# maksimt/rri_nmf

Measured on AMD Instinct MI355X. Metric: RRI sweeps/sec and achieved HBM GB/s on dense X (n x d, rank k), higher is better.
Workload: dtype f64

## Files before the change

### include/rri_hip.h

```cpp
#ifndef RRI_HIP_H
#define RRI_HIP_H

#include <stdint.h>
#include <stddef.h>

#ifdef __cplusplus
extern "C" {
#endif

#define RRI_ABI_VERSION 1
#define RRI_GRAM_SLICES 8
#define RRI_MAX_K 1024

typedef struct rri_ctx rri_ctx;
typedef struct rri_comm rri_comm;
#define RRI_COMM_ID_BYTES 128

typedef int32_t rri_status;
enum {
    RRI_OK = 0,
    RRI_PAUSED = 1,
    RRI_ERR_INVALID = -1,
    RRI_ERR_HIP = -2,
    RRI_ERR_UNSUPPORTED = -3,
// ... 92 lines not shown
rri_status rri_get_X_scales(rri_ctx* ctx, double* row_out, double* col_out);
rri_status rri_csr_column_positive_counts(rri_ctx* ctx, double* df_out);
rri_status rri_csr_scale_X(rri_ctx* ctx, const double* col_scale, int32_t normalize_rows, int64_t* zero_rows_out);

rri_status rri_comm_unique_id(uint8_t* id_out );
rri_status rri_comm_create(rri_comm** out, const uint8_t* id, int32_t rank, int32_t world, int32_t device);
typedef int32_t (*rri_allreduce_fn)(void* user, double* buf, int64_t count);
typedef int32_t (*rri_allgather_fn)(void* user, const double* send, int64_t count, double* recv);
typedef int32_t (*rri_broadcast_fn)(void* user, double* buf, int64_t count, int32_t root);
rri_status rri_comm_create_host(rri_comm** out, int32_t rank, int32_t world, rri_allreduce_fn allreduce,
                                rri_allgather_fn allgather, rri_broadcast_fn broadcast, void* user);
rri_status rri_comm_destroy(rri_comm* comm);
rri_status rri_attach_comm(rri_ctx* ctx, rri_comm* comm, int64_t row_offset, int64_t n_global);
rri_status rri_comm_broadcast(rri_ctx* ctx, double* host, int64_t count, int32_t root);
rri_status rri_comm_allreduce_sum(rri_ctx* ctx, double* host, int64_t count);
rri_status rri_comm_stats(rri_ctx* ctx, int32_t* rank, int32_t* world, int64_t* allreduce_calls);

rri_status rri_reduce_buffer(rri_ctx* ctx, void** dev_ptr, int64_t* n_elems);
rri_status rri_bind_reduce_buffer(rri_ctx* ctx, void* dev_ptr, int64_t n_elems);
rri_status rri_topic_reduce_local(rri_ctx* ctx, int32_t t);
rri_status rri_reduce_read(rri_ctx* ctx, double* out, int64_t count);
rri_status rri_reduce_write(rri_ctx* ctx, const double* in, int64_t count);
rri_status rri_topic_finish(rri_ctx* ctx, int32_t t);
rri_status rri_topic_finish_w(rri_ctx* ctx, int32_t t);
rri_status rri_resid_row_argmax(rri_ctx* ctx, double* value, int64_t* local_row);
rri_status rri_reset_row(rri_ctx* ctx, int64_t local_row, double* row_out_host);
rri_status rri_poll(rri_ctx* ctx);
rri_status rri_objective_parts(rri_ctx* ctx, double out[3]);

rri_status rri_timing_enable(rri_ctx* ctx, int32_t on);
rri_status rri_timing_read(rri_ctx* ctx, int32_t kernel_id, int64_t* launches, double* total_ms);
rri_status rri_synchronize(rri_ctx* ctx);
rri_status rri_onchip_info(rri_ctx* ctx, int32_t* eligible, int64_t* launches);
#define RRI_LAYOUT_FIELDS 23
rri_status rri_layout_info(rri_ctx* ctx, int64_t* out, int32_t n);
rri_status rri_onchip_fallbacks(rri_ctx* ctx, int64_t* fallbacks);
rri_status rri_device_memory(int64_t* buffers, int64_t* bytes);
rri_status rri_debug_xcc(rri_ctx* ctx, int32_t* out, int32_t count);
rri_status rri_sweep_until(rri_ctx* ctx, int32_t n_sweeps, double obj_prev, double stop_scale, double* obj_hist,
                           int32_t* sweeps_done);
rri_status rri_bench_rank1_update(rri_ctx* ctx, int32_t reps, double* avg_ms);
rri_status rri_bench_stream_copy(rri_ctx* ctx, int32_t reps, double* avg_ms);

#ifdef __cplusplus
}
#endif
#endif
```

### rri_nmf_amd/_capi.py

```python
import ctypes as C
import os

_PKG = os.path.dirname(os.path.abspath(__file__))
LIB_PATH = os.environ.get('RRI_HIP_LIB', os.path.join(_PKG, 'lib', 'librri_hip.so'))

RRI_GRAM_SLICES = 8
RRI_LAYOUT_FIELDS = 23
RRI_MAX_K = 1024
RRI_OK, RRI_PAUSED = 0, 1
RRI_ERR_INVALID, RRI_ERR_HIP, RRI_ERR_UNSUPPORTED = -1, -2, -3
RRI_ERR_UNBOUNDED, RRI_ERR_W_COL_ZERO, RRI_ERR_NOT_IMPLEMENTED, RRI_ERR_COMM = -4, -5, -6, -7
RRI_COMM_ID_BYTES = 128
RRI_F32, RRI_F64, RRI_F16 = 0, 1, 2
RRI_U8 = 4
RRI_UNWEIGHTED, RRI_WEIGHTED_DENSE, RRI_WEIGHTED_SPARSE, RRI_UNWEIGHTED_RESIDUAL, RRI_UNWEIGHTED_SPARSE = 0, 1, 2, 3, 4
RESET_NONE, RESET_MAX_RESID_DOCUMENT, RESET_RANDOM = 0, 1, 2
EVENT_NONE, EVENT_RESET_T, EVENT_RESET_W = 0, 1, 2
ABI_VERSION = 1


class Params(C.Structure):
    _fields_ = [('fix_W', C.c_int32), ('fix_T', C.c_int32), ('project_T_each_iter', C.c_int32),
                ('has_t_row_sum', C.c_int32), ('has_w_row_sum', C.c_int32), ('reset_method', C.c_int32),
                ('resets_left', C.c_int32), ('reserved0', C.c_int32),
                ('t_row_sum', C.c_double), ('w_row_sum', C.c_double),
                ('reg_w_l1', C.c_double), ('reg_w_l2', C.c_double), ('reg_t_l1', C.c_double),
                ('reg_t_l2', C.c_double), ('eps_div', C.c_double)]


class Event(C.Structure):
    _fields_ = [('kind', C.c_int32), ('topic', C.c_int32), ('sweep', C.c_int32), ('resume_topic', C.c_int32)]


_P = C.c_void_p
_I32, _I64, _D = C.c_int32, C.c_int64, C.c_double
ALLREDUCE_FN = C.CFUNCTYPE(C.c_int32, C.c_void_p, C.POINTER(C.c_double), C.c_int64)
ALLGATHER_FN = C.CFUNCTYPE(C.c_int32, C.c_void_p, C.POINTER(C.c_double), C.c_int64, C.POINTER(C.c_double))
BROADCAST_FN = C.CFUNCTYPE(C.c_int32, C.c_void_p, C.POINTER(C.c_double), C.c_int64, C.c_int32)
PROTOTYPES = {
    'rri_abi_version': (C.c_uint32, []),
# ... 137 lines not shown
```

### rri_nmf_amd/csrc/rri_hip.hip

```cpp
#include <hip/hip_runtime.h>
#include <dlfcn.h>
#include <rccl/rccl.h>

#include <algorithm>
#include <atomic>
#include <chrono>
#include <cstdarg>
#include <cstdio>
#include <mutex>
#include <cstdlib>
#include <cstring>
#include <string>
#include <utility>
#include <vector>

#include "rri_hip.h"
#include "rri_pick.hpp"
#include "rri_kernels.hpp"
#include "rri_wrri_kernels.hpp"
#include "rri_sparse_kernels.hpp"
#include "rri_onchip_kernels.hpp"

using namespace rri;

// ... 142 lines not shown
        unsigned short* idx = nullptr;
        void* val = nullptr;
        int* perm = nullptr;
        SpWork* work = nullptr;
    } sp[2];
    bool sparse_x = false;
    SpWork* spx_work = nullptr;
    double* rowhat = nullptr;
    double* Cpart = nullptr;
    double* N2part = nullptr;
    unsigned* Mcols = nullptr;
    bool nw_mask = false;
    bool mcols_tried = false;
    double mask_density = 1.0;
    int cpart_rows = 0;
    bool wcorr = false;
    int wcorr_topic = 0, wcorr_nrb = 0;
    bool resid_fresh = false;
    bool dt_pending = false;
    bool explicit_resid = false;
    bool dw_pending = false;
    int dw_topic = 0;
    double* told = nullptr;
    double *Gpart = nullptr, *tpart = nullptr, *rowobj = nullptr, *rowpos = nullptr, *normpart = nullptr;
    double *dtmp = nullptr;
    double* objbuf = nullptr;
    i64* itmp = nullptr;
    i64* tpart_idx = nullptr;
    double *resetT = nullptr, *resetW = nullptr;
    DevState* st = nullptr;

    int npanels = 1, rpb = 1, nrb = 1, nwb = 1, ntb = 1;
    int gpart_n = 1;
    int ttpart_n = 0;
    int xy_rows = 0;
    int xy_stride = 1;
    int ntb32 = 1;
    int tpart_n = 1;

    rri_params prm{};
    bool have_params = false, have_X = false, have_W = false, have_T = false, have_M = false;


    bool carry_valid = false;
    int carry_topic = -1;
    double* XYpart = nullptr;
    int xy_run = -1;
    bool xy_valid = false, x_sq_valid = false;
    bool obj_track_pending = false, obj_track_valid = false;
    double obj_track_value = 0.0;
    struct { bool active = false; double prev = 0.0, scale = 0.0; int n = 0; double* out = nullptr; } until;
    double *objhist = nullptr, *objdec = nullptr;
    double x_sq = 0.0;
    bool pending_wcheck = false;
    int pending_wcheck_topic = -1;

    bool paused = false;
    int run_total = 0;
    Cursor resume_at{0, 0, 0};
    bool resume_done = false;
    rri_event pending{RRI_EVENT_NONE, -1, 0, 0};

    bool resid_valid = false;
    bool skip_row_finish = false;
    int nwb256 = 1;

// ... 672 lines not shown
            typedef LaunchX<double> L;          \
            expr;                               \
        } else {                                \
            f16_unreachable(c);                 \
        }                                       \
    } while (0)
#define DISPATCH_RO(c, expr)                    \
    do {                                        \
        if ((c)->dtype == RRI_F32) {            \
            typedef LaunchX<float> L;           \
            expr;                               \
        } else if ((c)->dtype == RRI_F64) {     \
            typedef LaunchX<double> L;          \
            expr;                               \
        } else if ((c)->dtype == RRI_F16) {     \
            typedef LaunchX<_Float16> L;        \
            expr;                               \
        } else {                                \
            typedef LaunchX<unsigned char> L;   \
            expr;                               \
        }                                       \
    } while (0)

struct LK {
    static int gpart_rows(const rri_ctx* c) { return c->gpart_n; }
    template <bool UPDATE>
    static void wcol_resid(rri_ctx* c, int t, int tn, int sweep) {
        TimedScope ts(c, 1);
        hipLaunchKernelGGL((k_wcol_resid<UPDATE>), dim3(c->nwb256), dim3(256), 0, c->stream, c->W, c->ldw, (int)c->n,
                           c->k, t, tn, (const double*)c->Ypart, c->npanels, (const double*)c->Ttpart, c->nsplit,
                           c->dwv, c->Gpart, sweep, kparams(c), c->st);
        c->gpart_n = c->nwb256;
    }
    static size_t wcol_shmem(const rri_ctx* c) { return (size_t)(2 * c->k + 2 + 256 + 64) * sizeof(double); }
    template <bool UPDATE, bool CARRY>
    static void wcol_src(rri_ctx* c, int t, int tn, int sweep, const double* ypart, int nslices) {
        TimedScope ts(c, 1);
        hipLaunchKernelGGL((k_wcol<UPDATE, CARRY>), dim3(c->nwb), dim3(256), wcol_shmem(c), c->stream, c->W, c->ldw,
                           (int)c->n, c->k, t, tn, ypart, nslices, (const double*)c->Ttpart, c->ttpart_n, c->Gpart,
                           c->XYpart + (i64)t * c->xy_stride, sweep, kparams(c), c->st);
        c->gpart_n = c->nwb;
        if (UPDATE) note_xy(c, t, c->nwb * WCOL_TILES);
    }
    static void note_xy(rri_ctx* c, int t, int rows) {
        if (t == 0) { c->xy_run = 1; c->xy_rows = rows; }
        else c->xy_run = (c->xy_run == t && c->xy_rows == rows) ? t + 1 : -1;
        c->xy_valid = c->xy_run == c->k;
    }
    template <bool UPDATE, bool CARRY>
    static void wcol(rri_ctx* c, int t, int tn, int sweep) {
        wcol_src<UPDATE, CARRY>(c, t, tn, sweep, (const double*)c->Ypart, c->npanels);
    }
    static void reduce(rri_ctx* c) {
        const int nb = (int)((c->LD + 31) / 32) + GRAM_SLICES;
        hipLaunchKernelGGL(k_reduce, dim3(nb), dim3(1024), 0, c->stream, (const double*)c->Zpart, c->LD, c->nrb,
                           (const double*)c->Gpart, gpart_rows(c), c->k, c->red, (const DevState*)c->st);
    }
    static bool light(const rri_ctx* c) { return !(c->prm.project_T_each_iter && c->prm.has_t_row_sum); }
    static void trow(rri_ctx* c, int t, int check_prev, int tprev, int sweep, bool force_final) {
        hipLaunchKernelGGL(k_trow_numer, dim3(c->ntb), dim3(128), 0, c->stream, c->T, c->LD, (int)c->d, c->k, t,
                           (const double*)c->red, c->LD, c->xraw, c->tpart, c->tpart_idx, check_prev, tprev, sweep,
                           kparams(c), c->st, resid_sched(c) ? 1 : 0, resid_sched(c) ? c->told : (double*)nullptr);
        c->tpart_n = c->ntb;
        trow_final_if_needed(c, t, sweep, force_final);
    }
    static bool small(const rri_ctx* c) {
        return (double)gpart_rows(c) * (c->k + 2) * c->ntb32 <= 4.0e6;
    }
    static void trow_small(rri_ctx* c, int t, int check_prev, int tprev, int sweep, bool force_final) {
        hipLaunchKernelGGL(k_trow_small, dim3(c->ntb32), dim3(1024), 0, c->stream, c->T, c->LD, (int)c->d, c->k, t,
                           (const double*)c->Zpart, c->nrb, (const double*)c->Gpart, gpart_rows(c), c->red, c->LD, c->xraw,
                           c->tpart, c->tpart_idx, check_prev, tprev, sweep, kparams(c), c->st, resid_sched(c) ? 1 : 0,
                           resid_sched(c) ? c->told : (double*)nullptr);
        c->tpart_n = c->ntb32;
        trow_final_if_needed(c, t, sweep, force_final);
// ... 508 lines not shown
            if (c->sw.rot_debug) fprintf(stderr, "rri: tile rotation %d: %.4f ms per %s\n", rot, ms / 2.0f, what);
            if (best < 0.0f || ms < best) { best = ms; best_rot = rot; }
        }
        rot = best > 0.0f ? best_rot : 0;
        c->carry_valid = false;
        c->carry_topic = -1;
    };
    if (plain) {
        pick(c->rot_x, 2, "read-only pass", [&]() { DISPATCH_RO(c, (L::template pass<true, true>(c, 0, 0))); });
        return;
    }
    if (!c->resid_valid) {
        if (resid) r_refresh(c);
        else w_refresh(c);
    }
    auto null_update = [&]() {
        if (resid) {
            DISPATCH(c, {
                typename L::Upd u;
                u.a = c->zeros; u.b = c->zeros; u.a2 = c->zeros; u.b2 = c->zeros; u.b2sub = c->zeros;
                L::rank_update(c, c->E, c->LD, u, c->T, c->W);
            });
        } else {
            DISPATCH(c, (L::template wpass<true, true, true, true>(c, c->T, c->W, c->zeros, c->zeros, c->zeros, c->zeros)));
        }
    };
    pick(c->rot_r, c->sw.rot_cal > 1 ? std::min(c->sw.rot_cal, 8) : 2, "null update", null_update);
}

bool wsweep_ok(const rri_ctx* c) {
    return c->sw.wsweep && c->prm.fix_T && !c->prm.fix_W && !c->weighted && (!c->sparse || c->sparse_x) && c->k >= 1 &&
           c->k <= 256 && wsweep_lds_bytes(c->k) <= 150 * 1024;
}
static_assert(WCOL_TILES == 1, "enqueue_wsweep assumes one 64-row tile per k_wcol block");
bool enqueue_wsweep(rri_ctx* c, int sweep, int t0) {
    const int k = c->k;
    const size_t f8 = sizeof(double);
    if (dev_ensure(c, c->Gfull, (size_t)k * k * f8) != hipSuccess || dev_ensure(c, c->Wsweep0, (size_t)k * c->ldw * f8) != hipSuccess ||
        dev_ensure(c, c->wsum_part, (size_t)k * c->nwb * f8) != hipSuccess || dev_ensure(c, c->wsums, (size_t)k * f8) != hipSuccess)
        return false;
    if (allow_lds<k_wsweep_rows>(c, 152 * 1024) != hipSuccess) return false;
    flush_wcheck(c, sweep, t0);
    if (!c->q_valid) {
        DISPATCH_RO(c, L::xtt(c));
        c->q_valid = true;
    }
    if (!c->gfull_valid) {
        hipLaunchKernelGGL(k_gram, dim3(k, k), dim3(256), 0, c->stream, (const double*)c->T, c->LD, c->d, k, c->Gfull);
        c->gfull_valid = true;
    }
    {
        TimedScope ts(c, 1);
        hipLaunchKernelGGL(k_wsweep_rows, dim3(c->nwb), dim3(64), wsweep_lds_bytes(k), c->stream, c->W, c->Wsweep0, c->ldw, (int)c->n, k,
                           t0, (const double*)c->Qt, (const double*)c->Gfull, c->wsum_part, c->nwb, c->XYpart, (i64)c->xy_stride,
                           kparams(c), (const DevState*)c->st);
        if (!c->comm)
            hipLaunchKernelGGL(k_wsweep_verdict, dim3(1), dim3(1024), 0, c->stream, (const double*)c->wsum_part, c->nwb, c->wsums,
                               (const double*)c->Gfull, k, t0, sweep, 3, kparams(c), c->st);
        else {
            hipLaunchKernelGGL(k_wsweep_verdict, dim3(1), dim3(1024), 0, c->stream, (const double*)c->wsum_part, c->nwb, c->wsums,
                               (const double*)c->Gfull, k, t0, sweep, 1, kparams(c), c->st);
            comm_allreduce(c, c->wsums, k);
            hipLaunchKernelGGL(k_wsweep_verdict, dim3(1), dim3(1024), 0, c->stream, (const double*)c->wsum_part, c->nwb, c->wsums,
                               (const double*)c->Gfull, k, t0, sweep, 2, kparams(c), c->st);
        }
        hipLaunchKernelGGL(k_wsweep_repair, dim3((unsigned)((c->n + 255) / 256)), dim3(256), 0, c->stream, c->W, (const double*)c->Wsweep0,
                           c->ldw, (int)c->n, k, (const DevState*)c->st);
    }
    for (int t = t0; t < k; ++t) LK::note_xy(c, t, c->nwb * WCOL_TILES);
    c->skip_row_finish = false;
    c->carry_valid = false;
    changed(c, CH_W_COL);
    return true;
}

int pass_keep(const rri_ctx* c);
void xpack_release(rri_ctx* c) {
    dev_release(c, c->xp); dev_release(c, c->xp_flags); dev_release(c, c->xp_hmax);
    c->xp_valid = false;
    c->xp_flagged = c->xp_tiles = 0;
    c->xp_base = 0;
    c->keep_q = pass_keep(c);
}
void xpack_ensure(rri_ctx* c) {
    if (c->xp_done) return;
    if (wsweep_ok(c)) return;
    c->xp_done = true;
    c->xp_valid = false;
    c->keep_q = pass_keep(c);
    const bool reads_x = c->dtype == RRI_F32 && !c->weighted && !c->explicit_resid && !c->sparse && c->have_X;
    if (!reads_x || c->sw.x_pack == 0 || (c->sw.x_pack < 0 && c->keep_q < 0)) { xpack_release(c); return; }
    const i64 nitems = (c->n + xpack::ROWS - 1) / xpack::ROWS * c->npanels;
    if (dev_ensure(c, c->xp, (size_t)nitems * 4 * xpack::RECORD_BYTES) != hipSuccess || dev_ensure(c, c->xp_flags, (size_t)nitems) != hipSuccess ||
        dev_ensure(c, c->xp_hmax, sizeof(unsigned)) != hipSuccess) { xpack_release(c); return; }
    const int ncols = (int)std::min<i64>(c->ldx, c->LD);
    const unsigned grid = (unsigned)std::min<i64>(nitems, 8192);
    std::vector<unsigned char> flags((size_t)nitems);
    unsigned hmax = 0;
    (void)hipMemsetAsync(c->xp_hmax, 0, sizeof(unsigned), c->stream);
    (void)hipMemsetAsync(c->xp_flags, 0, (size_t)nitems, c->stream);
    hipLaunchKernelGGL(k_xpack_max, dim3(grid), dim3(256), 0, c->stream, (const float*)c->X, c->ldx, (int)c->n, ncols, c->npanels, nitems, c->xp_hmax);
    hipLaunchKernelGGL(k_xpack_encode, dim3(grid), dim3(256), 0, c->stream, (const float*)c->X, c->ldx, (int)c->n, ncols, c->npanels, nitems,
// ... 416 lines not shown
    i64 rpb = 0;
    {
        const bool rmw = explicit_resid || weighted == RRI_WEIGHTED_DENSE;
        const int total_max = weighted == RRI_WEIGHTED_DENSE ? 16384 : rmw ? 8192 : 1024;
        const i64 rows_min = weighted == RRI_WEIGHTED_DENSE ? 48 : rmw ? 96 : 192;
        for (int total = total_max; total >= 512 && rpb == 0; total -= 512) {
            const int nrb_t = std::max(1, total / c->npanels);
            const i64 r = (n + nrb_t - 1) / nrb_t;
            if (r >= rows_min || total == 512) rpb = r;
        }
    }
    rpb = std::max<i64>(rpb, 32);
    rpb = std::min<i64>(round_up(rpb, 16), rpb_cap);
    if (dtype == RRI_F32 && !weighted && !explicit_resid && !c->sparse) {
        rpb = c->sw.pk_rows > 0 ? std::min<i64>(round_up(std::max(c->sw.pk_rows, 16), 16), rpb_cap) : std::min<i64>(rpb, PK_ROWS_MAX);
        if (c->sw.pk_rows > 0) c->ro_il = c->sw.pk_il;
    }
    c->rpb = (int)rpb;
    c->nrb = (int)((n + rpb - 1) / rpb);
    if (c->sparse) {
        const i64 block_bytes = SP_BLOCK_BYTES;
        const i64 cap = sparse_x ? std::min<i64>(spx_block_cap(), std::max<i64>(64, (block_bytes / 8 - 64) / 64 * 64))
                                 : block_bytes / (3 * (i64)c->es);
        for (int w = 0; w < 2; ++w) {
            rri_ctx::SpCopy& cp = c->sp[w];
            cp.gdim = w == 0 ? d : n;
            cp.nseg = w == 0 ? n : d;
            cp.nblk = (int)((cp.gdim + cap - 1) / cap);
            cp.bw = (int)round_up((cp.gdim + cp.nblk - 1) / cp.nblk, 64);
        }
        c->npanels = c->sp[0].nblk;
        c->nrb = c->sp[1].nblk;
    }
    c->nwb = (int)((n + 64 * WCOL_TILES - 1) / (64 * WCOL_TILES));
    c->nwb256 = (int)((n + 255) / 256);
    c->ldw = n;
    c->keep_q = pass_keep(c);
    c->ntb = (int)((d + 127) / 128);
    c->ntb32 = (int)((c->LD + 31) / 32);
    c->tpart_n = c->ntb;
    c->nsplit = (int)std::max<i64>(1, std::min<i64>(8, d / 2048));
    c->red_elems = round_up(std::max<i64>(c->LD + (i64)GRAM_SLICES * (k + 2), weighted ? 2 * c->LD + 2 : 0), 4);

    const size_t f8 = sizeof(double);
    CR(dev_alloc(c, c->W, (size_t)k * c->ldw * f8));
    CR(dev_alloc(c, c->T, (size_t)k * c->LD * f8, true));
    CR(dev_alloc(c, c->Ypart, (size_t)c->npanels * n * f8, true));
    CR(dev_alloc(c, c->Zpart, (size_t)c->nrb * c->LD * f8, true));
    const size_t grows = (size_t)std::max(c->nwb, c->nrb);
    c->gpart_n = c->nwb;
    c->xy_stride = (int)std::max<size_t>(std::max<size_t>(grows, (size_t)c->nwb * WCOL_TILES), (size_t)std::max(c->n_cu, 1));
    CR(dev_alloc(c, c->Gpart, grows * (k + 2) * f8, true));
    CR(dev_alloc(c, c->XYpart, (size_t)k * c->xy_stride * f8, true));
    CR(dev_alloc(c, c->red, (size_t)c->red_elems * f8, true));
    CR(dev_alloc(c, c->xraw, (size_t)c->LD * f8, true));
    const size_t ttn = (size_t)std::max(c->nsplit, c->ntb32);
    c->ttpart_n = c->nsplit;
    CR(dev_alloc(c, c->Ttpart, ttn * k * f8, true));
    CR(dev_alloc(c, c->Qt, (size_t)k * c->ldw * f8));
    const size_t ntp = (size_t)std::max(c->ntb, c->ntb32);
    CR(dev_alloc(c, c->tpart, ntp * f8, true));
    CR(dev_alloc(c, c->tpart_idx, ntp * sizeof(i64)));
    CR(dev_alloc(c, c->normpart, 256 * 3 * f8));
    CR(dev_alloc(c, c->objbuf, (size_t)(2 * k * k + k) * f8));
    CR(dev_alloc(c, c->dtmp, 16 * f8));
    CR(dev_alloc(c, c->itmp, 16 * sizeof(i64)));
    const bool keeps_resid = explicit_resid || (weighted && !c->sparse);
    if (keeps_resid) CR(dev_alloc(c, c->E, (size_t)n * c->LD * c->es, c->LD != d));
    if (weighted) {
        CR(dev_alloc(c, c->Y2part, (size_t)c->npanels * n * f8, true));
        CR(dev_alloc(c, c->Z2part, (size_t)c->nrb * c->LD * f8, true));
        if (!c->sparse) {
            c->cpart_rows = (int)std::max<i64>(256, (n + 2047) / 2048);
            CR(dev_alloc(c, c->Cpart, (size_t)c->cpart_rows * c->LD * f8, true));
            CR(dev_alloc(c, c->N2part, (size_t)c->cpart_rows * c->LD * f8, true));
        }
        CR(dev_alloc(c, c->dtv, (size_t)c->LD * f8, true));
    }
    if (weighted || explicit_resid) CR(dev_alloc(c, c->dwv, (size_t)n * f8, explicit_resid));
    if (weighted) CR(dev_alloc(c, c->wold, (size_t)n * f8));
    if (explicit_resid) CR(dev_alloc(c, c->told, (size_t)c->LD * f8, true));
    if (weighted || explicit_resid) CR(dev_alloc(c, c->zeros, (size_t)std::max<i64>(c->LD, n) * f8, true));
    if (c->sparse) CR(dev_alloc(c, c->sp_Tt, (size_t)d * c->kp * f8, true));
    if (dtype == RRI_U8) {
// ... 1654 lines not shown
    if (c->comm_status != RRI_OK) { const rri_status r = c->comm_status; c->comm_status = RRI_OK; return r; }
    return RRI_OK;
}

rri_status rri_comm_stats(rri_ctx* c, int32_t* rank, int32_t* world, int64_t* allreduce_calls) {
    CHECK_CTX(c);
    if (rank) *rank = c->comm ? c->comm->rank : 0;
    if (world) *world = c->comm ? c->comm->world : 1;
    if (allreduce_calls) *allreduce_calls = c->comm ? c->comm->n_allreduce : 0;
    return RRI_OK;
}

rri_status rri_onchip_info(rri_ctx* c, int32_t* eligible, int64_t* launches) {
    CHECK_CTX(c);
    if (eligible) *eligible = (c->have_X && c->have_params && onchip_ok(c)) ? 1 : 0;
    if (launches) *launches = c->onchip_launches;
    return RRI_OK;
}

rri_status rri_layout_info(rri_ctx* c, int64_t* out, int32_t n) {
    CHECK_CTX(c);
    if (!out || n < 1) return fail(c, RRI_ERR_INVALID, "rri_layout_info needs room for at least one value");
    const bool dense_w = c->weighted == RRI_WEIGHTED_DENSE;
    const int64_t v[RRI_LAYOUT_FIELDS] = {
        c->sparse ? c->sp[0].nblk : 0, c->sparse ? c->sp[0].bw : 0, c->sparse ? c->sp[0].lps : 0, c->sparse ? c->sp[0].nwork : 0,
        c->sparse ? c->sp[1].nblk : 0, c->sparse ? c->sp[1].bw : 0, c->sparse ? c->sp[1].lps : 0, c->sparse ? c->sp[1].nwork : 0,
        c->rpb, c->nrb, c->npanels,
        c->Mbits ? 1 : 0, c->Mcols ? 1 : 0,
        c->mcols_tried && c->Mbits ? (int64_t)(c->mask_density * 1.0e9 + 0.5) : -1,
        dense_w && wtrow_small(c) ? 1 : 0,
        dense_w && c->nw_mask ? 1 : 0,
        !c->sparse && ro_pass_interleaved(c) ? 1 : 0,
        c->wcorr_nrb, c->n_cu,
        c->xp_valid ? 1 : 0, c->xp_valid ? c->xp_base : 0, c->xp_flagged, c->xp_tiles};
    for (int i = 0; i < n && i < RRI_LAYOUT_FIELDS; ++i) out[i] = v[i];
    return RRI_OK;
}

rri_status rri_device_memory(int64_t* buffers, int64_t* bytes) {
    if (buffers) *buffers = g_dev_buffers.load();
    if (bytes) *bytes = g_dev_bytes.load();
    return RRI_OK;
}

rri_status rri_debug_xcc(rri_ctx* c, int32_t* out, int32_t count) {
    CHECK_CTX(c);
    if (!out || count < 1 || count > 4096) return fail(c, RRI_ERR_INVALID, "bad count");
    HIPCHK(c, hipSetDevice(c->device));
    DevTmp dv;
    HIPCHK(c, dv.alloc((size_t)count * sizeof(int)));
    hipLaunchKernelGGL(k_xcc_probe, dim3((unsigned)count), dim3(64), 0, c->stream, (int*)dv.p);
    HIPCHK(c, hipMemcpyAsync(out, dv.p, (size_t)count * sizeof(int), hipMemcpyDeviceToHost, c->stream));
    HIPCHK(c, hipStreamSynchronize(c->stream));
    return RRI_OK;
}

rri_status rri_onchip_fallbacks(rri_ctx* c, int64_t* fallbacks) {
    CHECK_CTX(c);
    if (fallbacks) *fallbacks = c->onchip_fallbacks;
    return RRI_OK;
}

rri_status rri_timing_enable(rri_ctx* c, int32_t on) {
    CHECK_CTX(c);
    c->timing = on < 0 ? 0 : on;
    for (int i = 0; i < 4; ++i) c->timing_seq[i] = 0;
    return RRI_OK;
// ... 93 lines not shown
```

### rri_nmf_amd/csrc/rri_kernels.hpp

```cpp
#pragma once
#include <type_traits>

#include "rri_device.hpp"
#include "rri_halt.hpp"
#include "rri_hip.h"
#include "rri_xpack.hpp"

namespace rri {

typedef float f32x4 __attribute__((ext_vector_type(4)));
typedef double f64x2 __attribute__((ext_vector_type(2)));
typedef unsigned u32x4 __attribute__((ext_vector_type(4)));

template <typename SX> struct XVec;
template <> struct XVec<float> {
    typedef f32x4 type;
    static constexpr int N = 4;
    static __device__ __forceinline__ void unpack(const f32x4& v, double (&o)[4]) {
        o[0] = (double)v[0]; o[1] = (double)v[1]; o[2] = (double)v[2]; o[3] = (double)v[3];
    }
    static __device__ __forceinline__ f32x4 pack(const double (&o)[4]) {
        return f32x4{(float)o[0], (float)o[1], (float)o[2], (float)o[3]};
    }
    static __device__ __forceinline__ f32x4 zero() { return f32x4{0.f, 0.f, 0.f, 0.f}; }
// ... 439 lines not shown
    const i64 i = (i64)blockIdx.x * 256 + threadIdx.x;
    if (i >= n) return;
    double xs = 0.0;
    xs = ordered_sum<8>(Ypart + i, n, 0, npanels, 1);
    xs += 2.220446049250313e-16;
    inv[i] = xs < 1e-10 ? -1.0 : 1.0 / xs;
}

template <typename SX>
__global__ __launch_bounds__(256) void k_scale2d(SX* __restrict__ X, i64 ldx, i64 n, int d, const double* __restrict__ s,
                                                 const double* __restrict__ inv) {
    typedef XVec<SX> XV;
    typedef typename XV::type V;
    constexpr int VN = XV::N;
    const i64 vpr = ldx / VN, total = n * vpr;
    const double uniform = 1.0 / (double)d;
    for (i64 v = (i64)blockIdx.x * 256 + threadIdx.x; v < total; v += (i64)gridDim.x * 256) {
        const i64 i = v / vpr;
        const int j = (int)(v - i * vpr) * VN;
        V* p = reinterpret_cast<V*>(X + i * ldx + j);
        double xe[VN];
        XV::unpack(__builtin_nontemporal_load(p), xe);
        const double r = inv ? inv[i] : 1.0;
#pragma unroll
        for (int e = 0; e < VN; ++e) {
            if (j + e >= d) { xe[e] = 0.0; continue; }
            const double t = s ? xe[e] * s[j + e] : xe[e];
            xe[e] = r < 0.0 ? uniform : r * t;
        }
        __builtin_nontemporal_store(XV::pack(xe), p);
    }
}

constexpr int WCOL_TILES = 1;
constexpr int GRAM_SLICES = RRI_GRAM_SLICES;

template <bool UPDATE, bool CARRY>
__global__ __launch_bounds__(256) void k_wcol(double* __restrict__ Wt, i64 ldw, int n, int k, int t, int tn,
                                              const double* __restrict__ Ypart, int npanels,
                                              const double* __restrict__ Ttpart, int nsplit,
                                              double* __restrict__ Gpart, double* __restrict__ xyp, int sweep,
                                              KParams p, DevState* st) {
    if (st->halt) return;
    const int tid = threadIdx.x, lane = tid & 63, wave = tid >> 6;
    extern __shared__ __attribute__((aligned(16))) unsigned char smem[];
    double* tts = reinterpret_cast<double*>(smem);
    double* gsh = tts + k;
    double* dsh = gsh + k + 2;
    double* wsh = dsh + 256;
    double cden = 0.0;
    int mode = 0;
    for (int l = tid; l < k + 2; l += 256) gsh[l] = 0.0;
    if (UPDATE) {
        for (int l = tid; l < k; l += 256) {
            tts[l] = ordered_sum<8>(Ttpart + l, k, 0, nsplit, 1);
        }
        __syncthreads();
        cden = tts[t] + p.reg_w_l2;
        __syncthreads();
        if (tid == 0) tts[t] = 0.0;
        mode = wcol_denominator_mode(cden, p);
        if (mode < 0) {
            if (blockIdx.x == 0 && tid == 0) halt_set(st, mode, t, sweep, t);
            return;
        }
    }
    __syncthreads();
    constexpr int CH = 16;
    constexpr int TILES = WCOL_TILES;
    for (int tile = 0; tile < TILES; ++tile) {
        const i64 i = ((i64)blockIdx.x * TILES + tile) * 64 + lane;
        if (((i64)blockIdx.x * TILES + tile) * 64 >= n) break;
        const bool valid = i < n;
        const double wn = (CARRY && valid) ? Wt[(i64)tn * ldw + i] : 0.0;
        double y = 0.0;
        if (UPDATE && wave == 0 && valid) y = ordered_sum<8>(Ypart + i, n, 0, npanels, 1);
        double dotv = 0.0;
        for (int l0 = wave; l0 < k; l0 += 4 * CH) {
            double wl[CH];
#pragma unroll
            for (int q = 0; q < CH; ++q) {
                const int l = l0 + 4 * q;
                wl[q] = (l < k && valid && !(UPDATE && l == t)) ? Wt[(i64)l * ldw + i] : 0.0;
            }
#pragma unroll
            for (int q = 0; q < CH; ++q) {
                const int l = l0 + 4 * q;
                if (l < k) {
                    if (UPDATE) dotv = fma(wl[q], tts[l], dotv);
                    if (CARRY && !(UPDATE && l == t)) {
                        const double g = wave_sum<double>(wn * wl[q]);
                        if (lane == 0) gsh[l] += g;
                    }
                }
            }
        }
        double wnew = 0.0;
        if (UPDATE) {
            dsh[wave * 64 + lane] = dotv;
            __syncthreads();
            if (wave == 0) {
                const double dot = (dsh[lane] + dsh[64 + lane]) + (dsh[128 + lane] + dsh[192 + lane]);
                if (valid) {
                    const double numer = (y - dot) - p.reg_w_l1;
                    if (mode == 0) wnew = fmax(numer, 0.0) / (cden + p.eps);
                    else wnew = (-numer + cden < 0.0) ? p.w_row_sum : 0.0;
                    Wt[(i64)t * ldw + i] = wnew;
                }
                wsh[lane] = wnew;
            }
            __syncthreads();
            wnew = wsh[lane];
        }
        if (wave == 0) {
            const double nwp = wave_sum<double>(wn * wn);
            const double swp = wave_sum<double>(wnew);
            if (lane == 0) { gsh[k] += nwp; gsh[k + 1] += swp; }
            if (UPDATE) {
                const double xy = wave_sum<double>(wnew * y);
                if (lane == 0) xyp[(i64)blockIdx.x * TILES + tile] = xy;
            }
        } else if (wave == 1 && UPDATE && CARRY) {
            const double gt = wave_sum<double>(wn * wnew);
            if (lane == 0) gsh[t] += gt;
        }
        if (UPDATE) __syncthreads();
    }
    __syncthreads();
    double* gp = Gpart + (i64)blockIdx.x * (k + 2);
    for (int l = tid; l < k + 2; l += 256) gp[l] = gsh[l];
}

__host__ __device__ constexpr int wsweep_kp(int k) { return (k + 3) & ~3; }
__host__ __device__ constexpr size_t wsweep_lds_bytes(int k) { return ((size_t)k * wsweep_kp(k) + 64 * (size_t)k) * sizeof(double); }

__global__ __launch_bounds__(64) void k_wsweep_rows(double* __restrict__ Wt, double* __restrict__ Wprev, i64 ldw, int n, int k,
                                                    int t0, const double* __restrict__ Qt, const double* __restrict__ G,
                                                    double* __restrict__ colsum, int nwb, double* __restrict__ xyp,
                                                    i64 xy_stride, KParams p, const DevState* __restrict__ st) {
    if (st->halt) return;
    extern __shared__ __attribute__((aligned(16))) unsigned char smem[];
    const int kp = wsweep_kp(k);
    double* gsh = reinterpret_cast<double*>(smem);
    double* wsh = gsh + (size_t)k * kp;
    const int lane = threadIdx.x;
    const i64 i = (i64)blockIdx.x * 64 + lane;
    const bool valid = i < n;
    for (int q = lane; q < k * kp; q += 64) {
        const int l = q / kp, c = q - l * kp;
        gsh[q] = c < k ? G[(i64)l * k + c] : 0.0;
    }
    constexpr int CH = 8;
    for (int l0 = 0; l0 < k; l0 += CH) {
        double wv[CH];
#pragma unroll
        for (int q = 0; q < CH; ++q) wv[q] = (l0 + q < k && valid) ? Wt[(i64)(l0 + q) * ldw + i] : 0.0;
#pragma unroll
        for (int q = 0; q < CH; ++q) {
            const int l = l0 + q;
// ... 166 lines not shown
        if (tid < 32 && j < ldz) {
            double s = 0.0;
            for (int q = 0; q < 32; ++q) s += sh[q * 33 + tid];
            red[j] = s;
        }
    } else {
        const int gs = blockIdx.x - nzb;
        const int per = (nwb + GRAM_SLICES - 1) / GRAM_SLICES;
        const int b0 = gs * per, b1 = min(nwb, b0 + per);
        const int lane = tid & 63, wave = tid >> 6;
        for (int l0 = 0; l0 < k + 2; l0 += 64) {
            const int l = l0 + lane;
            double a = 0.0;
            if (l < k + 2) a = ordered_sum<8>(Gpart + l, k + 2, b0 + wave, b1, 16);
            __syncthreads();
            sh[wave * 64 + lane] = a;
            __syncthreads();
            if (wave == 0 && l < k + 2) {
                double s = 0.0;
                for (int q = 0; q < 16; ++q) s += sh[q * 64 + lane];
                red[ldz + (i64)gs * (k + 2) + l] = s;
            }
        }
    }
}

__device__ __forceinline__ double red_gram(const double* __restrict__ red, i64 ldz, int k, int l) {
    double s = 0.0;
#pragma unroll
    for (int g = 0; g < GRAM_SLICES; ++g) s += red[ldz + (i64)g * (k + 2) + l];
    return s;
}

__global__ __launch_bounds__(128) void k_trow_numer(double* __restrict__ T, i64 ldt, int d, int k, int t,
                                                    const double* __restrict__ red, i64 ldz,
                                                    double* __restrict__ xraw, double* __restrict__ tpart,
                                                    i64* __restrict__ tpart_idx, int check_prev, int tprev,
                                                    int sweep, KParams p, DevState* st, int resid_form,
                                                    double* __restrict__ told) {
    if (st->halt) return;
    const int tid = threadIdx.x;
    __shared__ double scratch[40];
    __shared__ double gsh[RRI_MAX_K];
    const double nw = red_gram(red, ldz, k, k);
    if (check_prev) {
        const int code = wcol_code(red_gram(red, ldz, k, k + 1), p);
        if (code != 0) {
            if (blockIdx.x == 0 && tid == 0) halt_set(st, code, tprev, sweep, t);
            return;
        }
    }
    const double c = nw + p.reg_t_l2;
    const bool project = p.project_T && p.has_trs;
    const int mode = trow_denominator_mode(c, p);
    if (mode < 0) {
        if (blockIdx.x == 0 && tid == 0) halt_set(st, mode, t, sweep, t);
        return;
    }
    for (int l = tid; l < k; l += 128) gsh[l] = (l == t) ? (resid_form ? -nw : 0.0) : red_gram(red, ldz, k, l);
    __syncthreads();
    const i64 j = (i64)blockIdx.x * 128 + tid;
    double x = 0.0, mx = -1.0e300;
    if (j < d) {
        if (told) told[j] = T[(i64)t * ldt + j];
        double a0 = 0.0, a1 = 0.0, a2 = 0.0, a3 = 0.0;
        for (int l0 = 0; l0 < k; l0 += 16) {
            double tv[16];
#pragma unroll
            for (int q = 0; q < 16; ++q) tv[q] = (l0 + q < k) ? T[(i64)(l0 + q) * ldt + j] : 0.0;
#pragma unroll
            for (int q = 0; q < 16; q += 4) {
                if (l0 + q < k) a0 = fma(gsh[l0 + q], tv[q], a0);
                if (l0 + q + 1 < k) a1 = fma(gsh[l0 + q + 1], tv[q + 1], a1);
                if (l0 + q + 2 < k) a2 = fma(gsh[l0 + q + 2], tv[q + 2], a2);
                if (l0 + q + 3 < k) a3 = fma(gsh[l0 + q + 3], tv[q + 3], a3);
            }
        }
        const double acc = (a0 + a1) + (a2 + a3);
        const double numer = (red[j] - acc) - p.reg_t_l1;
        if (mode == 0) x = fmax(numer, 0.0) / (c + p.eps);
        else if (mode == 1) x = (-numer + c < 0.0) ? p.t_row_sum : 0.0;
        else { x = numer; mx = numer; }
        xraw[j] = x;
        if (mode == 1 || (mode == 0 && !project)) T[(i64)t * ldt + j] = x;
    }
    if (mode != 2) {
        const double s = block_sum(x, scratch);
        if (tid == 0) tpart[blockIdx.x] = s;
    } else {
        i64 idx = (j < d) ? j : (i64)0x7fffffffffffffffLL;
        wave_argmax(mx, idx);
        __shared__ double wm[2];
        __shared__ i64 wi[2];
        if ((tid & 63) == 0) { wm[tid >> 6] = mx; wi[tid >> 6] = idx; }
        __syncthreads();
        if (tid == 0) {
            if (wm[1] > wm[0] || (wm[1] == wm[0] && wi[1] < wi[0])) { wm[0] = wm[1]; wi[0] = wi[1]; }
            tpart[blockIdx.x] = wm[0];
            tpart_idx[blockIdx.x] = wi[0];
        }
    }
    if (blockIdx.x == 0 && tid == 0) st->tmode = mode;
}

__global__ __launch_bounds__(1024) void k_trow_small(double* __restrict__ T, i64 ldt, int d, int k, int t,
                                                     const double* __restrict__ Zpart, int nrb,
                                                     const double* __restrict__ Gpart, int nwb, double* __restrict__ red,
                                                     i64 ldz, double* __restrict__ xraw, double* __restrict__ tpart,
                                                     i64* __restrict__ tpart_idx, int check_prev, int tprev, int sweep,
                                                     KParams p, DevState* st, int resid_form, double* __restrict__ told) {
    if (st->halt) return;
    const int tid = threadIdx.x;
// ... 967 lines not shown
```

### rri_nmf_amd/engine.py

```python
import ctypes as C
import re

import numpy as np

from . import _capi
from ._capi import Params, Event

EPS_DIV = float(np.spacing(10))

_NP2RRI = {np.dtype(np.float32): _capi.RRI_F32, np.dtype(np.float64): _capi.RRI_F64, np.dtype(np.float16): _capi.RRI_F16,
           np.dtype(np.uint8): _capi.RRI_U8}
_READ_ONLY = (np.dtype(np.float16), np.dtype(np.uint8))
_HOST_TYPES = (np.dtype(np.float32), np.dtype(np.float64))
_RESET_CODES = {None: _capi.RESET_NONE, 'max_resid_document': _capi.RESET_MAX_RESID_DOCUMENT,
                'random': _capi.RESET_RANDOM}


class ZeroTotalRows(ValueError):

    def __init__(self, count):
        ValueError.__init__(self, '%d row(s) of X sum to less than 1e-10: normalisation would make them dense (1/d), which an X '
                                  'kept as CSR or as counts cannot hold; X was left unchanged' % count)
        self.count = int(count)

# ... 593 lines not shown
    def resid_row_argmax(self):
        val, row = C.c_double(0.0), C.c_int64(-1)
        self._check(self._lib.rri_resid_row_argmax(self._h, C.byref(val), C.byref(row)))
        return float(val.value), int(row.value)

    def reset_row(self, local_row):
        out = np.empty(self.d, dtype=np.float64)
        self._check(self._lib.rri_reset_row(self._h, int(local_row), out.ctypes.data_as(C.POINTER(C.c_double))))
        return out

    def apply_reset_vectors(self, t, T_row, W_col):
        T_row = np.ascontiguousarray(T_row, dtype=np.float64)
        W_col = np.ascontiguousarray(W_col, dtype=np.float64)
        self._check(self._lib.rri_apply_reset_vectors(
            self._h, int(t), T_row.ctypes.data_as(C.POINTER(C.c_double)),
            W_col.ctypes.data_as(C.POINTER(C.c_double))))
        self.n_resets_used += 1

    def timing_enable(self, on=True, every=1):
        self._check(self._lib.rri_timing_enable(self._h, int(every) if on else 0))

    def timing_read(self, kernel_id):
        cnt, ms = C.c_int64(0), C.c_double(0.0)
        self._check(self._lib.rri_timing_read(self._h, int(kernel_id), C.byref(cnt), C.byref(ms)))
        return int(cnt.value), float(ms.value)

    def onchip_info(self):
        el, n = C.c_int32(0), C.c_int64(0)
        self._check(self._lib.rri_onchip_info(self._h, C.byref(el), C.byref(n)))
        return bool(el.value), int(n.value)

    LAYOUT_COPY_FIELDS = ('nblk', 'bw', 'lps', 'nwork')
    LAYOUT_FIELDS = ('rpb', 'nrb', 'npanels', 'mask_bits', 'mask_cols', 'mask_density', 'wtrow_small', 'nw_from_mask',
                     'interleaved', 'wcorr_nrb', 'n_cu', 'x_pack', 'x_pack_base', 'x_pack_flagged', 'x_pack_tiles')
    assert 2 * len(LAYOUT_COPY_FIELDS) + len(LAYOUT_FIELDS) == _capi.RRI_LAYOUT_FIELDS

    def layout_info(self):
        nc = len(self.LAYOUT_COPY_FIELDS)
        out = (C.c_int64 * _capi.RRI_LAYOUT_FIELDS)()
        self._check(self._lib.rri_layout_info(self._h, out, _capi.RRI_LAYOUT_FIELDS))
        v = [int(x) for x in out]
        info = {name: (v[i], v[nc + i]) for i, name in enumerate(self.LAYOUT_COPY_FIELDS)}
        info.update(zip(self.LAYOUT_FIELDS, v[2 * nc:]))
        for name in ('mask_bits', 'mask_cols', 'wtrow_small', 'nw_from_mask', 'interleaved', 'x_pack'):
            info[name] = bool(info[name])
        info['mask_density'] = None if info['mask_density'] < 0 else info['mask_density'] * 1e-9
        return info

    def debug_xcc(self, count=32):
        out = (C.c_int32 * count)()
        self._check(self._lib.rri_debug_xcc(self._h, out, count))
        return list(out)

    def onchip_fallbacks(self):
        n = C.c_int64(0)
        self._check(self._lib.rri_onchip_fallbacks(self._h, C.byref(n)))
        return int(n.value)

    def sweep_until(self, n_sweeps, obj_prev, stop_scale):
        n_sweeps = int(n_sweeps)
        if not self.onchip_info()[0]:
            return None
        hist = np.full(n_sweeps, np.nan, dtype=np.float64)
        done = C.c_int32(0)
        st = self._lib.rri_sweep_until(self._h, n_sweeps, float(obj_prev), float(stop_scale),
                                       hist.ctypes.data_as(C.POINTER(C.c_double)), C.byref(done))
        if st == _capi.RRI_ERR_UNSUPPORTED:
# ... 17 lines not shown
```

Baseline: 33.89.

## Hoist global loads ahead of halt check and barriers in wcol and trow kernels

k_wcol and k_trow_numer now issue their global loads (Ttpart, Ypart panels, the first W/T rows, gram slices) into registers before reading the halt flag and before the first barrier. This overlaps memory latency with the setup and reduction phases. The Ypart panel sums are staged through LDS across all four waves rather than summed by wave 0 alone. The change also drops the WCOL_TILES abstraction, adds an occupancy query for k_wcol, and exposes three new layout fields, at the cost of more registers and LDS per block.

```diff
diff --git a/include/rri_hip.h b/include/rri_hip.h
--- a/include/rri_hip.h
+++ b/include/rri_hip.h
@@ -148,7 +148,7 @@
 rri_status rri_timing_read(rri_ctx* ctx, int32_t kernel_id, int64_t* launches, double* total_ms);
 rri_status rri_synchronize(rri_ctx* ctx);
 rri_status rri_onchip_info(rri_ctx* ctx, int32_t* eligible, int64_t* launches);
-#define RRI_LAYOUT_FIELDS 23
+#define RRI_LAYOUT_FIELDS 26
 rri_status rri_layout_info(rri_ctx* ctx, int64_t* out, int32_t n);
 rri_status rri_onchip_fallbacks(rri_ctx* ctx, int64_t* fallbacks);
 rri_status rri_device_memory(int64_t* buffers, int64_t* bytes);
diff --git a/rri_nmf_amd/_capi.py b/rri_nmf_amd/_capi.py
--- a/rri_nmf_amd/_capi.py
+++ b/rri_nmf_amd/_capi.py
@@ -5,7 +5,7 @@
 LIB_PATH = os.environ.get('RRI_HIP_LIB', os.path.join(_PKG, 'lib', 'librri_hip.so'))
 
 RRI_GRAM_SLICES = 8
-RRI_LAYOUT_FIELDS = 23
+RRI_LAYOUT_FIELDS = 26
 RRI_MAX_K = 1024
 RRI_OK, RRI_PAUSED = 0, 1
 RRI_ERR_INVALID, RRI_ERR_HIP, RRI_ERR_UNSUPPORTED = -1, -2, -3
diff --git a/rri_nmf_amd/csrc/rri_hip.hip b/rri_nmf_amd/csrc/rri_hip.hip
--- a/rri_nmf_amd/csrc/rri_hip.hip
+++ b/rri_nmf_amd/csrc/rri_hip.hip
@@ -198,6 +198,7 @@
 
     int npanels = 1, rpb = 1, nrb = 1, nwb = 1, ntb = 1;
     int gpart_n = 1;
+    int wcol_resident = 0;
     int ttpart_n = 0;
     int xy_rows = 0;
     int xy_stride = 1;
@@ -936,7 +937,15 @@
                            c->dwv, c->Gpart, sweep, kparams(c), c->st);
         c->gpart_n = c->nwb256;
     }
-    static size_t wcol_shmem(const rri_ctx* c) { return (size_t)(2 * c->k + 2 + 256 + 64) * sizeof(double); }
+    static size_t wcol_shmem(const rri_ctx* c) { return (size_t)wcol_lds_doubles(c->k) * sizeof(double); }
+    static void wcol_residency(rri_ctx* c) {
+        int b = 0;
+        if (hipOccupancyMaxActiveBlocksPerMultiprocessor(&b, k_wcol<true, true>, 256, wcol_shmem(c)) != hipSuccess) {
+            (void)hipGetLastError();
+            b = 0;
+        }
+        c->wcol_resident = std::max(b, 0) * std::max(c->n_cu, 1);
+    }
     template <bool UPDATE, bool CARRY>
     static void wcol_src(rri_ctx* c, int t, int tn, int sweep, const double* ypart, int nslices) {
         TimedScope ts(c, 1);
@@ -944,7 +953,7 @@
                            (int)c->n, c->k, t, tn, ypart, nslices, (const double*)c->Ttpart, c->ttpart_n, c->Gpart,
                            c->XYpart + (i64)t * c->xy_stride, sweep, kparams(c), c->st);
         c->gpart_n = c->nwb;
-        if (UPDATE) note_xy(c, t, c->nwb * WCOL_TILES);
+        if (UPDATE) note_xy(c, t, c->nwb);
     }
     static void note_xy(rri_ctx* c, int t, int rows) {
         if (t == 0) { c->xy_run = 1; c->xy_rows = rows; }
@@ -1519,7 +1528,6 @@
     return c->sw.wsweep && c->prm.fix_T && !c->prm.fix_W && !c->weighted && (!c->sparse || c->sparse_x) && c->k >= 1 &&
            c->k <= 256 && wsweep_lds_bytes(c->k) <= 150 * 1024;
 }
-static_assert(WCOL_TILES == 1, "enqueue_wsweep assumes one 64-row tile per k_wcol block");
 bool enqueue_wsweep(rri_ctx* c, int sweep, int t0) {
     const int k = c->k;
     const size_t f8 = sizeof(double);
@@ -1554,7 +1562,7 @@
         hipLaunchKernelGGL(k_wsweep_repair, dim3((unsigned)((c->n + 255) / 256)), dim3(256), 0, c->stream, c->W, (const double*)c->Wsweep0,
                            c->ldw, (int)c->n, k, (const DevState*)c->st);
     }
-    for (int t = t0; t < k; ++t) LK::note_xy(c, t, c->nwb * WCOL_TILES);
+    for (int t = t0; t < k; ++t) LK::note_xy(c, t, c->nwb);
     c->skip_row_finish = false;
     c->carry_valid = false;
     changed(c, CH_W_COL);
@@ -2037,7 +2045,8 @@
         c->npanels = c->sp[0].nblk;
         c->nrb = c->sp[1].nblk;
     }
-    c->nwb = (int)((n + 64 * WCOL_TILES - 1) / (64 * WCOL_TILES));
+    c->nwb = (int)((n + 63) / 64);
+    LK::wcol_residency(c);
     c->nwb256 = (int)((n + 255) / 256);
     c->ldw = n;
     c->keep_q = pass_keep(c);
@@ -2054,7 +2063,7 @@
     CR(dev_alloc(c, c->Zpart, (size_t)c->nrb * c->LD * f8, true));
     const size_t grows = (size_t)std::max(c->nwb, c->nrb);
     c->gpart_n = c->nwb;
-    c->xy_stride = (int)std::max<size_t>(std::max<size_t>(grows, (size_t)c->nwb * WCOL_TILES), (size_t)std::max(c->n_cu, 1));
+    c->xy_stride = (int)std::max<size_t>(grows, (size_t)std::max(c->n_cu, 1));
     CR(dev_alloc(c, c->Gpart, grows * (k + 2) * f8, true));
     CR(dev_alloc(c, c->XYpart, (size_t)k * c->xy_stride * f8, true));
     CR(dev_alloc(c, c->red, (size_t)c->red_elems * f8, true));
@@ -3775,7 +3784,8 @@
         dense_w && c->nw_mask ? 1 : 0,
         !c->sparse && ro_pass_interleaved(c) ? 1 : 0,
         c->wcorr_nrb, c->n_cu,
-        c->xp_valid ? 1 : 0, c->xp_valid ? c->xp_base : 0, c->xp_flagged, c->xp_tiles};
+        c->xp_valid ? 1 : 0, c->xp_valid ? c->xp_base : 0, c->xp_flagged, c->xp_tiles,
+        1, c->nwb, c->wcol_resident};
     for (int i = 0; i < n && i < RRI_LAYOUT_FIELDS; ++i) out[i] = v[i];
     return RRI_OK;
 }
diff --git a/rri_nmf_amd/csrc/rri_kernels.hpp b/rri_nmf_amd/csrc/rri_kernels.hpp
--- a/rri_nmf_amd/csrc/rri_kernels.hpp
+++ b/rri_nmf_amd/csrc/rri_kernels.hpp
@@ -495,8 +495,10 @@
     }
 }
 
-constexpr int WCOL_TILES = 1;
+constexpr int WCOL_YP = 16;
 constexpr int GRAM_SLICES = RRI_GRAM_SLICES;
+
+__host__ __device__ constexpr int wcol_lds_doubles(int k) { return 2 * k + 2 + 256 + 64 + WCOL_YP * 64; }
 
 template <bool UPDATE, bool CARRY>
 __global__ __launch_bounds__(256) void k_wcol(double* __restrict__ Wt, i64 ldw, int n, int k, int t, int tn,
@@ -504,21 +506,65 @@
                                               const double* __restrict__ Ttpart, int nsplit,
                                               double* __restrict__ Gpart, double* __restrict__ xyp, int sweep,
                                               KParams p, DevState* st) {
-    if (st->halt) return;
-    const int tid = threadIdx.x, lane = tid & 63, wave = tid >> 6;
+    const int halted = st->halt;
+    const int tid = threadIdx.x, lane = tid & 63;
+    const int wave = __builtin_amdgcn_readfirstlane(tid >> 6);
     extern __shared__ __attribute__((aligned(16))) unsigned char smem[];
     double* tts = reinterpret_cast<double*>(smem);
     double* gsh = tts + k;
     double* dsh = gsh + k + 2;
     double* wsh = dsh + 256;
+    double* ysh = wsh + 64;
+    constexpr int CH = 16;
+    const i64 base = (i64)blockIdx.x * 64;
+    const bool valid = base + lane < n;
+    const int lo = valid ? lane : 0;
+    double ttv[8];
+    if (UPDATE) {
+        const int tc = tid < k ? tid : 0;
+#pragma unroll
+        for (int q = 0; q < 8; ++q) ttv[q] = Ttpart[(i64)(q < nsplit ? q : 0) * k + tc];
+    }
+    double wn = CARRY ? (Wt + ((i64)tn * ldw + base))[lo] : 0.0;
+    double yv[WCOL_YP / 4], wl[CH];
+    if (UPDATE) {
+#pragma unroll
+        for (int q = 0; q < WCOL_YP / 4; ++q) {
+            const int pn = wave * (WCOL_YP / 4) + q;
+            yv[q] = (Ypart + ((i64)(pn < npanels ? pn : 0) * n + base))[lo];
+        }
+    }
+#pragma unroll
+    for (int q0 = 0; q0 < CH; q0 += 4) {
+        if (wave + 4 * q0 < k) {
+#pragma unroll
+            for (int q = q0; q < q0 + 4; ++q) {
+                const int l = wave + 4 * q;
+                wl[q] = (Wt + ((i64)(l < k ? l : 0) * ldw + base))[lo];
+            }
+        } else {
+#pragma unroll
+            for (int q = q0; q < q0 + 4; ++q) wl[q] = 0.0;
+        }
+    }
+    wn = valid ? wn : 0.0;
     double cden = 0.0;
     int mode = 0;
     for (int l = tid; l < k + 2; l += 256) gsh[l] = 0.0;
     if (UPDATE) {
-        for (int l = tid; l < k; l += 256) {
-            tts[l] = ordered_sum<8>(Ttpart + l, k, 0, nsplit, 1);
-        }
-        __syncthreads();
+        {
+            double a = 0.0;
+#pragma unroll
+            for (int q = 0; q < 8; ++q) a += q < nsplit ? ttv[q] : 0.0;
+            if (tid < k) tts[tid] = nsplit > 8 ? ordered_sum_acc<8>(a, Ttpart + tid, k, 8, nsplit, 1) : a;
+        }
+        for (int l = tid + 256; l < k; l += 256) tts[l] = ordered_sum<8>(Ttpart + l, k, 0, nsplit, 1);
+#pragma unroll
+        for (int q = 0; q < WCOL_YP / 4; ++q) ysh[(wave * (WCOL_YP / 4) + q) * 64 + lane] = valid ? yv[q] : 0.0;
+    }
+    __syncthreads();
+    if (halted) return;
+    if (UPDATE) {
         cden = tts[t] + p.reg_w_l2;
         __syncthreads();
         if (tid == 0) tts[t] = 0.0;
@@ -527,67 +573,61 @@
             if (blockIdx.x == 0 && tid == 0) halt_set(st, mode, t, sweep, t);
             return;
         }
-    }
-    __syncthreads();
-    constexpr int CH = 16;
-    constexpr int TILES = WCOL_TILES;
-    for (int tile = 0; tile < TILES; ++tile) {
-        const i64 i = ((i64)blockIdx.x * TILES + tile) * 64 + lane;
-        if (((i64)blockIdx.x * TILES + tile) * 64 >= n) break;
-        const bool valid = i < n;
-        const double wn = (CARRY && valid) ? Wt[(i64)tn * ldw + i] : 0.0;
-        double y = 0.0;
-        if (UPDATE && wave == 0 && valid) y = ordered_sum<8>(Ypart + i, n, 0, npanels, 1);
-        double dotv = 0.0;
-        for (int l0 = wave; l0 < k; l0 += 4 * CH) {
-            double wl[CH];
+        __syncthreads();
+    }
+    double dotv = 0.0;
+    for (int l0 = wave; l0 < k; l0 += 4 * CH) {
+        if (l0 != wave) {
 #pragma unroll
             for (int q = 0; q < CH; ++q) {
                 const int l = l0 + 4 * q;
-                wl[q] = (l < k && valid && !(UPDATE && l == t)) ? Wt[(i64)l * ldw + i] : 0.0;
-            }
-#pragma unroll
-            for (int q = 0; q < CH; ++q) {
-                const int l = l0 + 4 * q;
-                if (l < k) {
-                    if (UPDATE) dotv = fma(wl[q], tts[l], dotv);
-                    if (CARRY && !(UPDATE && l == t)) {
-                        const double g = wave_sum<double>(wn * wl[q]);
-                        if (lane == 0) gsh[l] += g;
-                    }
+                wl[q] = (Wt + ((i64)(l < k ? l : 0) * ldw + base))[lo];
+            }
+        }
+#pragma unroll
+        for (int q = 0; q < CH; ++q) {
+            const int l = l0 + 4 * q;
+            if (l < k) {
+                const double w = (valid && !(UPDATE && l == t)) ? wl[q] : 0.0;
+                if (UPDATE) dotv = fma(w, tts[l], dotv);
+                if (CARRY && !(UPDATE && l == t)) {
+                    const double g = wave_sum<double>(wn * w);
+                    if (lane == 0) gsh[l] += g;
                 }
             }
         }
-        double wnew = 0.0;
+    }
+    double wnew = 0.0, y = 0.0;
+    if (UPDATE) {
+        dsh[wave * 64 + lane] = dotv;
+        __syncthreads();
+        if (wave == 0) {
+            const int np0 = npanels < WCOL_YP ? npanels : WCOL_YP;
+            for (int pn = 0; pn < np0; ++pn) y += ysh[pn * 64 + lane];
+            if (npanels > WCOL_YP && valid) y = ordered_sum_acc<8>(y, Ypart + base + lane, n, WCOL_YP, npanels, 1);
+            const double dot = (dsh[lane] + dsh[64 + lane]) + (dsh[128 + lane] + dsh[192 + lane]);
+            if (valid) {
+                const double numer = (y - dot) - p.reg_w_l1;
+                if (mode == 0) wnew = fmax(numer, 0.0) / (cden + p.eps);
+                else wnew = (-numer + cden < 0.0) ? p.w_row_sum : 0.0;
+                (Wt + ((i64)t * ldw + base))[lane] = wnew;
+            }
+            wsh[lane] = wnew;
+        }
+        __syncthreads();
+        wnew = wsh[lane];
+    }
+    if (wave == 0) {
+        const double nwp = wave_sum<double>(wn * wn);
+        const double swp = wave_sum<double>(wnew);
+        if (lane == 0) { gsh[k] += nwp; gsh[k + 1] += swp; }
         if (UPDATE) {
-            dsh[wave * 64 + lane] = dotv;
-            __syncthreads();
-            if (wave == 0) {
-                const double dot = (dsh[lane] + dsh[64 + lane]) + (dsh[128 + lane] + dsh[192 + lane]);
-                if (valid) {
-                    const double numer = (y - dot) - p.reg_w_l1;
-                    if (mode == 0) wnew = fmax(numer, 0.0) / (cden + p.eps);
-                    else wnew = (-numer + cden < 0.0) ? p.w_row_sum : 0.0;
-                    Wt[(i64)t * ldw + i] = wnew;
-                }
-                wsh[lane] = wnew;
-            }
-            __syncthreads();
-            wnew = wsh[lane];
-        }
-        if (wave == 0) {
-            const double nwp = wave_sum<double>(wn * wn);
-            const double swp = wave_sum<double>(wnew);
-            if (lane == 0) { gsh[k] += nwp; gsh[k + 1] += swp; }
-            if (UPDATE) {
-                const double xy = wave_sum<double>(wnew * y);
-                if (lane == 0) xyp[(i64)blockIdx.x * TILES + tile] = xy;
-            }
-        } else if (wave == 1 && UPDATE && CARRY) {
-            const double gt = wave_sum<double>(wn * wnew);
-            if (lane == 0) gsh[t] += gt;
-        }
-        if (UPDATE) __syncthreads();
+            const double xy = wave_sum<double>(wnew * y);
+            if (lane == 0) xyp[blockIdx.x] = xy;
+        }
+    } else if (wave == 1 && UPDATE && CARRY) {
+        const double gt = wave_sum<double>(wn * wnew);
+        if (lane == 0) gsh[t] += gt;
     }
     __syncthreads();
     double* gp = Gpart + (i64)blockIdx.x * (k + 2);
@@ -820,19 +860,60 @@
     return s;
 }
 
+constexpr int TROW_PRE = 64;
+constexpr int TROW_CH = 32;
+
 __global__ __launch_bounds__(128) void k_trow_numer(double* __restrict__ T, i64 ldt, int d, int k, int t,
                                                     const double* __restrict__ red, i64 ldz,
                                                     double* __restrict__ xraw, double* __restrict__ tpart,
                                                     i64* __restrict__ tpart_idx, int check_prev, int tprev,
                                                     int sweep, KParams p, DevState* st, int resid_form,
                                                     double* __restrict__ told) {
-    if (st->halt) return;
+    const int halted = st->halt;
     const int tid = threadIdx.x;
     __shared__ double scratch[40];
     __shared__ double gsh[RRI_MAX_K];
-    const double nw = red_gram(red, ldz, k, k);
+    const i64 j = (i64)blockIdx.x * 128 + tid;
+    const bool on = j < d;
+    double gn[GRAM_SLICES], gc[GRAM_SLICES], gl[GRAM_SLICES];
+#pragma unroll
+    for (int g = 0; g < GRAM_SLICES; ++g) {
+        gn[g] = red[ldz + (i64)g * (k + 2) + k];
+        gc[g] = red[ldz + (i64)g * (k + 2) + k + 1];
+        gl[g] = red[ldz + (i64)g * (k + 2) + (tid < k ? tid : 0)];
+    }
+    const double rj = red[on ? j : (i64)d - 1];
+    double tv[TROW_PRE];
+    {
+        const double* tp = T + (on ? j : (i64)d - 1);
+#pragma unroll
+        for (int q0 = 0; q0 < TROW_PRE; q0 += 16) {
+            if (q0 < k) {
+#pragma unroll
+                for (int q = q0; q < q0 + 16; ++q) tv[q] = tp[(i64)min(q, k - 1) * ldt];
+            } else {
+#pragma unroll
+                for (int q = q0; q < q0 + 16; ++q) tv[q] = 0.0;
+            }
+        }
+    }
+    double nw = 0.0;
+#pragma unroll
+    for (int g = 0; g < GRAM_SLICES; ++g) nw += gn[g];
+    {
+        double s = 0.0;
+#pragma unroll
+        for (int g = 0; g < GRAM_SLICES; ++g) s += gl[g];
+        if (tid < k) gsh[tid] = (tid == t) ? (resid_form ? -nw : 0.0) : s;
+    }
+    for (int l = tid + 128; l < k; l += 128) gsh[l] = (l == t) ? (resid_form ? -nw : 0.0) : red_gram(red, ldz, k, l);
+    __syncthreads();
+    if (halted) return;
     if (check_prev) {
-        const int code = wcol_code(red_gram(red, ldz, k, k + 1), p);
+        double cs = 0.0;
+#pragma unroll
+        for (int g = 0; g < GRAM_SLICES; ++g) cs += gc[g];
+        const int code = wcol_code(cs, p);
         if (code != 0) {
             if (blockIdx.x == 0 && tid == 0) halt_set(st, code, tprev, sweep, t);
             return;
@@ -845,27 +926,31 @@
         if (blockIdx.x == 0 && tid == 0) halt_set(st, mode, t, sweep, t);
         return;
     }
-    for (int l = tid; l < k; l += 128) gsh[l] = (l == t) ? (resid_form ? -nw : 0.0) : red_gram(red, ldz, k, l);
-    __syncthreads();
-    const i64 j = (i64)blockIdx.x * 128 + tid;
     double x = 0.0, mx = -1.0e300;
-    if (j < d) {
+    if (on) {
         if (told) told[j] = T[(i64)t * ldt + j];
         double a0 = 0.0, a1 = 0.0, a2 = 0.0, a3 = 0.0;
-        for (int l0 = 0; l0 < k; l0 += 16) {
-            double tv[16];
-#pragma unroll
-            for (int q = 0; q < 16; ++q) tv[q] = (l0 + q < k) ? T[(i64)(l0 + q) * ldt + j] : 0.0;
-#pragma unroll
-            for (int q = 0; q < 16; q += 4) {
-                if (l0 + q < k) a0 = fma(gsh[l0 + q], tv[q], a0);
-                if (l0 + q + 1 < k) a1 = fma(gsh[l0 + q + 1], tv[q + 1], a1);
-                if (l0 + q + 2 < k) a2 = fma(gsh[l0 + q + 2], tv[q + 2], a2);
-                if (l0 + q + 3 < k) a3 = fma(gsh[l0 + q + 3], tv[q + 3], a3);
+#pragma unroll
+        for (int q = 0; q < TROW_PRE; q += 4) {
+            if (q < k) a0 = fma(gsh[q], tv[q], a0);
+            if (q + 1 < k) a1 = fma(gsh[q + 1], tv[q + 1], a1);
+            if (q + 2 < k) a2 = fma(gsh[q + 2], tv[q + 2], a2);
+            if (q + 3 < k) a3 = fma(gsh[q + 3], tv[q + 3], a3);
+        }
+        for (int l0 = TROW_PRE; l0 < k; l0 += TROW_CH) {
+            double tw[TROW_CH];
+#pragma unroll
+            for (int q = 0; q < TROW_CH; ++q) tw[q] = (l0 + q < k) ? T[(i64)(l0 + q) * ldt + j] : 0.0;
+#pragma unroll
+            for (int q = 0; q < TROW_CH; q += 4) {
+                if (l0 + q < k) a0 = fma(gsh[l0 + q], tw[q], a0);
+                if (l0 + q + 1 < k) a1 = fma(gsh[l0 + q + 1], tw[q + 1], a1);
+                if (l0 + q + 2 < k) a2 = fma(gsh[l0 + q + 2], tw[q + 2], a2);
+                if (l0 + q + 3 < k) a3 = fma(gsh[l0 + q + 3], tw[q + 3], a3);
             }
         }
         const double acc = (a0 + a1) + (a2 + a3);
-        const double numer = (red[j] - acc) - p.reg_t_l1;
+        const double numer = (rj - acc) - p.reg_t_l1;
         if (mode == 0) x = fmax(numer, 0.0) / (c + p.eps);
         else if (mode == 1) x = (-numer + c < 0.0) ? p.t_row_sum : 0.0;
         else { x = numer; mx = numer; }
diff --git a/rri_nmf_amd/engine.py b/rri_nmf_amd/engine.py
--- a/rri_nmf_amd/engine.py
+++ b/rri_nmf_amd/engine.py
@@ -649,7 +649,8 @@
 
     LAYOUT_COPY_FIELDS = ('nblk', 'bw', 'lps', 'nwork')
     LAYOUT_FIELDS = ('rpb', 'nrb', 'npanels', 'mask_bits', 'mask_cols', 'mask_density', 'wtrow_small', 'nw_from_mask',
-                     'interleaved', 'wcorr_nrb', 'n_cu', 'x_pack', 'x_pack_base', 'x_pack_flagged', 'x_pack_tiles')
+                     'interleaved', 'wcorr_nrb', 'n_cu', 'x_pack', 'x_pack_base', 'x_pack_flagged', 'x_pack_tiles',
+                     'wcol_tiles', 'wcol_grid', 'wcol_resident')
     assert 2 * len(LAYOUT_COPY_FIELDS) + len(LAYOUT_FIELDS) == _capi.RRI_LAYOUT_FIELDS
 
     def layout_info(self):
```

New measurement: 34.19, median of 6. About the same (+0.9%).
